# Boese0601/Dyadic-Interaction-Modeling

Measured on AMD Instinct MI355X. Metric: listener clips/sec (T=300, EMOCA-56), higher is better.
Workload: dtype bf16; 1 GPU; C3: B=256/GPU synthetic dyad clips, T=300, SLMFT.forward(mode='val'): listener VQ encode + encoder + 299-step AR decode (top-k 52 sampling) + VQ decode; global_batch=256, seq_len=300, gather=tokens+coeffs, gather_bytes_per_rank=17452032

## Files before the change

dyadic-interaction-modeling_amd/csrc/common.hpp:

```cpp
#pragma once
#include <hip/hip_runtime.h>
#include <stdint.h>
#include <stdio.h>
#include <string.h>
#include <string>

#include "../../include/dimx.h"

namespace dimx {

void set_error(const char* fmt, ...);
const char* get_error();

#define DIMX_HIP(expr)                                                                       \
    do {                                                                                     \
        hipError_t _e = (expr);                                                              \
        if (_e != hipSuccess) {                                                              \
            dimx::set_error("%s:%d: %s -> %s", __FILE__, __LINE__, #expr, hipGetErrorString(_e)); \
            return DIMX_ERR_HIP;                                                             \
        }                                                                                    \
    } while (0)

#define DIMX_REQUIRE(cond, code, ...)       \
    do {                                    \
// ... 362 lines not shown
int lstm_bwd_run(const float* dy, const float* save, const float* const* w_hh, int B, int T, float* dgates, void* scratch,
                 size_t scratch_bytes, int flags, int cu_count, int* fault_count, hipStream_t st);
int launch_context_concat(int out_dtype, const float* x_s, const float* patch, const float* audio, void* ctx,
                          int M, int dim, int dim_a, hipStream_t s);
int launch_finalize_idx(int32_t* idx, const int32_t* lens, int B, int T, int32_t pad_value, hipStream_t s,
                        int fqn = 1);
int launch_shift_tokens(const int32_t* z, int32_t* inp, int32_t* tgt, int B, int T, hipStream_t s);
int launch_ce_argmax(const float* logits, const int32_t* target, float* row_loss, int32_t* argmax_tok, int R,
                     int V, hipStream_t s);
int launch_sample(const float* logits, int ld_logits, int R, int top_k, float temperature, const float* noise,
                  uint64_t seed, const int32_t* step_dev, uint64_t step_host, int32_t* tokens, int tok_ld,
                  int tok_col_from_step, int nslab, long slab_stride, float* logits_out, int logits_out_ld, int row0,
                  int rows_total, const float* emb_table, int emb_C, float* x_next, int32_t* step_rw, unsigned* done_ctr,
                  hipStream_t s, const float* pos_table = nullptr, float pos_scale = 0.f, int pos_rows = 0,
                  const int32_t* dev_params = nullptr,
                  void* y_next = nullptr, const float* y_gamma = nullptr, int y_dtype = DIMX_F32);
int launch_gen_params(int32_t* base, int groups, float temperature, uint64_t seed, int row_off, int rows_total,
                      hipStream_t s);
int launch_embed_step(const float* table, int C, int rows, const int32_t* start, const int32_t* tokens, int tok_ld,
                      const int32_t* step_dev, float* x, int B, int start_div, hipStream_t s,
                      const float* pos_table = nullptr, float pos_scale = 0.f);
int launch_add_pos_rows(float* x, const float* pos, int M, int n, int C, float scale, hipStream_t s);
int launch_mask_lens(const uint8_t* mask, int32_t* lens, int B, int T, hipStream_t s);
int launch_legacy_scramble(int out_dtype, const float* E, const int32_t* idx, const int32_t* lens, void* out, int B,
                           int T, int fqn, int zdim, int n_embed, hipStream_t s);
int launch_step_inc(int32_t* step_dev, hipStream_t s);
int launch_copy_rows_step(const float* src, float* dst, int B, int V, int n, const int32_t* step_dev, hipStream_t s);
int launch_mask_and(const uint8_t* a, const uint8_t* b, uint8_t* out, int n, hipStream_t s);

}
```

dyadic-interaction-modeling_amd/csrc/elementwise.hip:

```cpp
#include "common.hpp"

namespace dimx {
namespace {

template <typename OutT>
__global__ void cast_pad_kernel(const float* __restrict__ x, int ldx, const float* __restrict__ coladd,
                                OutT* __restrict__ y, int ldy, int M, int K, const uint8_t* __restrict__ zero_rows) {
    const long total = (long)M * ldy;
    for (long i = (long)blockIdx.x * blockDim.x + threadIdx.x; i < total; i += (long)gridDim.x * blockDim.x) {
        const int m = (int)(i / ldy), k = (int)(i - (long)m * ldy);
        float v = 0.f;
        if (k < K && !(zero_rows && zero_rows[m])) {
            v = x[(size_t)m * ldx + k];
            if (coladd) v += coladd[k];
        }
        store_from_f32<OutT>(y + i, v);
    }
}

template <typename OutT>
__global__ void gather_rows_kernel(const float* __restrict__ table, int ld_table, int rows,
                                   const int32_t* __restrict__ idx, OutT* __restrict__ y, int ldy, int M, int C) {
    const long total = (long)M * C;
    for (long i = (long)blockIdx.x * blockDim.x + threadIdx.x; i < total; i += (long)gridDim.x * blockDim.x) {
// ... 79 lines not shown
}

__global__ __launch_bounds__(256) void sample_kernel(const float* __restrict__ logits, int ld, int R, int top_k,
                                                     float temperature, const float* __restrict__ noise,
                                                     uint64_t seed, const int32_t* __restrict__ step_dev,
                                                     uint64_t step_host, int32_t* __restrict__ tokens, int tok_ld,
                                                     int tok_col_from_step, int nslab, long slab_stride,
                                                     float* __restrict__ logits_out, int logits_out_ld, int row0,
                                                     int rows_total,
                                                     const float* __restrict__ emb_table, int emb_C,
                                                     float* __restrict__ x_next, int32_t* __restrict__ step_rw,
                                                     unsigned* __restrict__ done_ctr,
                                                     const float* __restrict__ pos_table, float pos_scale,
                                                     int pos_rows, const int32_t* __restrict__ dev_params,
                                                     void* __restrict__ y_next, const float* __restrict__ y_gamma,
                                                     int y_bf16) {
    const int row = blockIdx.x * (blockDim.x >> 6) + (threadIdx.x >> 6), lane = threadIdx.x & 63;
    const uint64_t step = step_dev ? (uint64_t)*step_dev : step_host;
    if (dev_params) {
        temperature = __builtin_bit_cast(float, dev_params[0]);
        seed = *(const uint64_t*)(dev_params + 2);
    }
    const int rng_off = dev_params ? dev_params[4] : 0;
    const int rng_tot = dev_params && dev_params[5] > 0 ? dev_params[5] : rows_total;
    if (row < R) {
    const float* lr = logits + (size_t)row * ld;
    float2 gam[16];
    const bool fast_embed = x_next && emb_C / 2 <= 16 * 64;
    if (y_next && fast_embed) {
#pragma unroll
        for (int k = 0; k < 16; ++k) {
// ... 113 lines not shown
        tok = bi;
    }
    if (lane == 0) tokens[(size_t)row * tok_ld + (tok_col_from_step ? (int)step : 0)] = tok;
    if (x_next) {
        const float2* src = (const float2*)(emb_table + (size_t)tok * emb_C);
        float2* dst = (float2*)(x_next + (size_t)row * emb_C);
        const bool with_pos = pos_table && (int)step + 1 < pos_rows;
        const float2* pr = with_pos ? (const float2*)(pos_table + (size_t)(step + 1) * emb_C) : nullptr;
        const int nv = emb_C / 2;
        if (nv <= 16 * 64) {
            float2 v[16];
#pragma unroll
            for (int k = 0; k < 16; ++k) {
                const int i = lane + 64 * k;
                v[k] = src[i < nv ? i : nv - 1];
            }
            if (with_pos) {
                float2 q[16];
#pragma unroll
                for (int k = 0; k < 16; ++k) {
                    const int i = lane + 64 * k;
                    q[k] = pr[i < nv ? i : nv - 1];
                }
#pragma unroll
                for (int k = 0; k < 16; ++k)
                    v[k] = make_float2(__fadd_rn(v[k].x, __fmul_rn(q[k].x, pos_scale)), __fadd_rn(v[k].y, __fmul_rn(q[k].y, pos_scale)));
            }
#pragma unroll
            for (int k = 0; k < 16; ++k) {
                const int i = lane + 64 * k;
// ... 63 lines not shown
    tok = tok < 0 ? 0 : (tok >= rows ? rows - 1 : tok);
    const float4* src = (const float4*)(table + (size_t)tok * C);
    float4* dst = (float4*)(x + (size_t)b * C);
    if (pos_table) {
        const float4* pr = (const float4*)(pos_table + (size_t)step * C);
        for (int i = threadIdx.x; i < C / 4; i += blockDim.x) {
            const float4 e = src[i], q = pr[i];
            dst[i] = make_float4(__fadd_rn(e.x, __fmul_rn(q.x, pos_scale)), __fadd_rn(e.y, __fmul_rn(q.y, pos_scale)),
                                 __fadd_rn(e.z, __fmul_rn(q.z, pos_scale)), __fadd_rn(e.w, __fmul_rn(q.w, pos_scale)));
        }
    } else {
        for (int i = threadIdx.x; i < C / 4; i += blockDim.x) dst[i] = src[i];
    }
}

__global__ void add_pos_rows_kernel(float* __restrict__ x, const float* __restrict__ pos, int M, int n, int C,
                                    float scale) {
    const long total = (long)M * C;
    for (long i = (long)blockIdx.x * blockDim.x + threadIdx.x; i < total; i += (long)gridDim.x * blockDim.x) {
        const int m = (int)(i / C), c = (int)(i - (long)m * C);
        x[i] = __fadd_rn(x[i], __fmul_rn(pos[(size_t)(m % n) * C + c], scale));
    }
}

__global__ __launch_bounds__(64) void mask_lens_kernel(const uint8_t* __restrict__ mask, int32_t* __restrict__ lens,
                                                       int T) {
    const int b = blockIdx.x;
    int n = 0;
    for (int t = threadIdx.x; t < T; t += 64) n += mask[(size_t)b * T + t] ? 1 : 0;
#pragma unroll
// ... 114 lines not shown

int launch_ce_argmax(const float* logits, const int32_t* target, float* row_loss, int32_t* argmax_tok, int R, int V,
                     hipStream_t s) {
    DIMX_REQUIRE(V == 512, DIMX_ERR_ARG, "ce_argmax: vocabulary %d != 512", V);
    hipLaunchKernelGGL(ce_argmax_kernel, dim3(ceil_div(R, 4)), dim3(256), 0, s, logits, target, row_loss, argmax_tok,
                       R);
    DIMX_HIP(hipGetLastError());
    return DIMX_OK;
}

int launch_sample(const float* logits, int ld_logits, int R, int top_k, float temperature, const float* noise,
                  uint64_t seed, const int32_t* step_dev, uint64_t step_host, int32_t* tokens, int tok_ld,
                  int tok_col_from_step, int nslab, long slab_stride, float* logits_out, int logits_out_ld, int row0,
                  int rows_total, const float* emb_table, int emb_C, float* x_next, int32_t* step_rw, unsigned* done_ctr,
                  hipStream_t s, const float* pos_table, float pos_scale, int pos_rows, const int32_t* dev_params,
                  void* y_next, const float* y_gamma, int y_dtype) {
    DIMX_REQUIRE(logits && tokens && R > 0, DIMX_ERR_ARG, "sample: bad arguments");
    DIMX_REQUIRE(!y_next || (x_next && y_gamma && emb_C % 128 == 0 && emb_C <= 2048), DIMX_ERR_ARG,
                 "sample: the fused pre-norm needs the fused embedding and a width of k * 128 <= 2048");
    const int wpb = R <= 1024 ? 1 : 4;
    hipLaunchKernelGGL(sample_kernel, dim3(ceil_div(R, wpb)), dim3(64 * wpb), 0, s, logits, ld_logits, R, top_k,
                       temperature, noise, seed, step_dev, step_host, tokens, tok_ld, tok_col_from_step, nslab < 1 ? 1 : nslab,
                       slab_stride, logits_out, logits_out_ld, row0, rows_total, emb_table, emb_C, x_next, step_rw, done_ctr,
                       pos_table, pos_scale, pos_rows, dev_params, y_next, y_gamma, y_dtype == DIMX_BF16 ? 1 : 0);
    DIMX_HIP(hipGetLastError());
    return DIMX_OK;
}

int launch_gen_params(int32_t* base, int groups, float temperature, uint64_t seed, int row_off, int rows_total,
                      hipStream_t s) {
    hipLaunchKernelGGL(gen_params_kernel, dim3(1), dim3(64), 0, s, base, groups, temperature, seed, row_off, rows_total);
    DIMX_HIP(hipGetLastError());
    return DIMX_OK;
}

int launch_embed_step(const float* table, int C, int rows, const int32_t* start, const int32_t* tokens, int tok_ld,
                      const int32_t* step_dev, float* x, int B, int start_div, hipStream_t s, const float* pos_table,
                      float pos_scale) {
    DIMX_REQUIRE(C % 4 == 0, DIMX_ERR_ARG, "embed_step: C %% 4");
    hipLaunchKernelGGL(embed_step_kernel, dim3(B), dim3(256), 0, s, table, C, start, tokens, tok_ld, step_dev, x,
                       rows, start_div < 1 ? 1 : start_div, pos_table, pos_scale);
    DIMX_HIP(hipGetLastError());
    return DIMX_OK;
}

int launch_add_pos_rows(float* x, const float* pos, int M, int n, int C, float scale, hipStream_t s) {
    DIMX_REQUIRE(x && pos && M > 0 && n > 0, DIMX_ERR_ARG, "add_pos_rows: bad arguments");
    const long total = (long)M * C;
    const int blocks = (int)(total / 256 + 1 < 4096 ? total / 256 + 1 : 4096);
    hipLaunchKernelGGL(add_pos_rows_kernel, dim3(blocks), dim3(256), 0, s, x, pos, M, n, C, scale);
    DIMX_HIP(hipGetLastError());
    return DIMX_OK;
}

int launch_mask_lens(const uint8_t* mask, int32_t* lens, int B, int T, hipStream_t s) {
    DIMX_REQUIRE(mask && lens && B > 0 && T > 0, DIMX_ERR_ARG, "mask_lens: bad arguments");
// ... 40 lines not shown
```

dyadic-interaction-modeling_amd/csrc/model.hip:

```cpp
#include <stdarg.h>
#include <stdlib.h>
#include <set>

#include "model.hpp"

namespace dimx {

static thread_local char g_err[1024] = "";
void set_error(const char* fmt, ...) {
    va_list ap;
    va_start(ap, fmt);
    vsnprintf(g_err, sizeof(g_err), fmt, ap);
    va_end(ap);
}
const char* get_error() { return g_err; }

static std::string vq_prefix(int which) { return which == 0 ? "speaker_vq." : "listener_vq."; }

struct KeySpec {
    std::string name;
    std::vector<int64_t> shape;
};

static void vq_keys(const dimx_dims& d, int which, std::vector<KeySpec>& out) {
// ... 387 lines not shown
    DIMX_TRY(pack_linear(c, {pre + "project_in.weight"}, c->host.count(pre + "project_in.bias") ? pre + "project_in.bias" : "", false,
                         &e->proj_in));
    DIMX_TRY(upload_f32(c, pre + "pos_emb.emb.weight", &e->pos_emb));
    for (int i = 0; i < c->encg[0].depth; ++i) {
        DIMX_TRY(pack_xattn(c, xl(pre, 2 * i), false, &e->attn[i]));
        DIMX_TRY(pack_xff(c, xl(pre, 2 * i + 1), &e->ff[i]));
    }
    DIMX_TRY(upload_f32(c, pre + "attn_layers.final_norm.weight", &e->final_g));
    return DIMX_OK;
}

static void free_packed(dimx_ctx* c) {
    for (void* p : c->dev_allocs) (void)hipFree(p);
    c->dev_allocs.clear();
    c->packed_mask = 0;
}

enum { COMP_VQ0 = 1, COMP_VQ1 = 2, COMP_ENC = 4, COMP_DEC = 8, COMP_ALL = 15, COMP_MESH = 16 };

static std::vector<KeySpec> comp_keys(const dimx_dims& d, int comp) {
    std::vector<KeySpec> k;
    if (comp == COMP_MESH) {
        mesh_keys(d, k);
        return k;
    }
    if (d.variant == 1) {
        if (comp == COMP_VQ0) legacy_speaker_vq_keys(d, k);
        if (comp == COMP_VQ1) vq_keys(d, 1, k);
        if (comp == COMP_ENC) xenc_keys(d, "generator.encoder.", (int64_t)d.spk_face_quan_num * d.vq_zdim, k);
        if (comp == COMP_DEC) {
// ... 100 lines not shown
        }
        if (comp == COMP_MESH) {
            const std::string p = "vertice_map_reverse_lstm.";
            for (int l = 0; l < 2; ++l)
                for (int dir = 0; dir < 2; ++dir) {
                    const std::string sfx = "_l" + std::to_string(l) + lstm_suffix(dir);
                    DIMX_TRY(upload_f32(c, p + "weight_ih" + sfx, &c->mesh.w_ih[l][dir]));
                    DIMX_TRY(upload_f32(c, p + "weight_hh" + sfx, &c->mesh.w_hh[l][dir]));
                    DIMX_TRY(upload_f32(c, p + "bias_ih" + sfx, &c->mesh.b_ih[l][dir]));
                    DIMX_TRY(upload_f32(c, p + "bias_hh" + sfx, &c->mesh.b_hh[l][dir]));
                }
            DIMX_TRY(pack_linear(c, {"vertice_map_reverse.0.weight"}, "vertice_map_reverse.0.bias", false, &c->mesh.l1));
            DIMX_TRY(pack_linear(c, {"vertice_map_reverse.2.weight"}, "vertice_map_reverse.2.bias", false, &c->mesh.l2));
        }
        c->packed_mask |= comp;
    }
    c->graph_valid = false;
    return DIMX_OK;
}

int vq_pe_buffers(dimx_ctx* c, int which, const float** pe_enc, const float** pe_dec) {
    DIMX_REQUIRE(which == 0 || which == 1, DIMX_ERR_ARG, "vq_pe_buffers: which must be 0 or 1");
    DIMX_HIP(hipSetDevice(c->device));
    DIMX_TRY(ensure_packed(c, which == 0 ? COMP_VQ0 : COMP_VQ1));
    *pe_enc = c->vq[which].pe_enc;
    *pe_dec = c->vq[which].pe_dec;
    return DIMX_OK;
}

static inline size_t es_of(const dimx_ctx* c) { return dtype_size(c->at); }
// ... 263 lines not shown
        c->encg[0] = c->encg[1] = {din, din, d.dim, d.heads, d.dim_head, d.enc_depth, d.ff_mult, 0};
        c->decg = {d.dim, d.heads, d.dim_head, d.dec_depth, d.ff_mult, 1, d.num_tokens, d.dim};
    } else {
        const int causal = d.variant == 2 ? 0 : 1, abs_pos = d.variant == 2 ? 1 : 0;
        c->encg[0] = {d.dim_in, 64, d.dim, d.heads, d.dim_head, d.enc_depth, d.ff_mult, causal};
        c->encg[1] = {d.dim, d.dim, d.dim, d.heads, d.dim_head, d.enc_depth, d.ff_mult, causal};
        c->decg = {d.dim + d.dim_a, d.heads, d.dim_head, d.dec_depth, d.ff_mult, abs_pos, d.num_tokens, d.dim + d.dim_a};
    }
    for (const auto& k : all_keys(d)) c->required.push_back(k.name);
    const char* ng = getenv("DIMX_NO_GRAPH");
    c->use_graph = (ng && ng[0] == '1') ? 0 : 1;
    const char* nc = getenv("DIMX_NO_CHAIN");
    c->use_chain = (nc && nc[0] == '1') ? 0 : 1;
    c->use_layer_chain = getenv("DIMX_NO_LAYER_CHAIN") ? 0 : 1;
    c->multi_tr = getenv("DIMX_NO_MULTI_TR") ? 0 : 1;
    if (getenv("DIMX_LAYER_PROF")) {
        void* p = nullptr;
        if (hipMalloc(&p, (size_t)8 * 256 * 16 * 8) == hipSuccess) {
            (void)hipMemset(p, 0, (size_t)8 * 256 * 16 * 8);
            c->layer_prof_dev = (unsigned long long*)p;
        }
    }
    if (const char* pg = getenv("DIMX_PREFILL_GROUPS")) {
        const int v = atoi(pg);
        if (v >= 1 && v <= dimx_ctx::kPreGroups) c->prefill_groups = v;
    }
    {
        int cus = 0;
        if (hipDeviceGetAttribute(&cus, hipDeviceAttributeMultiprocessorCount, device_id) == hipSuccess) c->cu_count = cus;
    }
// ... 11 lines not shown
        if (h->graph_exec[g]) (void)hipGraphExecDestroy(h->graph_exec[g]);
        if (h->grp_stream[g]) (void)hipStreamDestroy(h->grp_stream[g]);
        if (h->ev_join[g]) (void)hipEventDestroy(h->ev_join[g]);
    }
    if (h->ev_fork) (void)hipEventDestroy(h->ev_fork);
    for (int g = 0; g < dimx_ctx::kPreGroups - 1; ++g) {
        if (h->pre_stream[g]) (void)hipStreamDestroy(h->pre_stream[g]);
        if (h->pre_join[g]) (void)hipEventDestroy(h->pre_join[g]);
    }
    if (h->pre_fork) (void)hipEventDestroy(h->pre_fork);
    if (h->cap_stream) (void)hipStreamDestroy(h->cap_stream);
    if (h->chain_err_ev) (void)hipEventDestroy(h->chain_err_ev);
    if (h->chain_err_dev) (void)hipFree(h->chain_err_dev);
    if (h->chain_stats_dev) (void)hipFree(h->chain_stats_dev);
    if (h->layer_prof_dev) (void)hipFree(h->layer_prof_dev);
    if (h->chain_err_host) (void)hipHostFree(h->chain_err_host);
    free_packed(h);
    train_forget(h);
    delete h;
    return DIMX_OK;
}

int dimx_numeric_mode(dimx_handle h) { return h ? h->mode : DIMX_ERR_ARG; }

int dimx_set_shard(dimx_handle h, int row_offset, int rows_total) {
    DIMX_REQUIRE(h, DIMX_ERR_ARG, "set_shard: null handle");
    DIMX_REQUIRE(row_offset >= 0 && (rows_total == 0 || rows_total > row_offset), DIMX_ERR_ARG,
                 "set_shard: row_offset %d, rows_total %d", row_offset, rows_total);
    h->shard_row_off = row_offset;
    h->shard_rows_total = rows_total;
// ... 871 lines not shown
    const XAttn& sa = h->dec.self_[0];
    const XAttn& ca = h->dec.cross[0];
    c.g1.W = sa.out.w; c.g1.N = sa.out.N; c.g1.K = sa.out.K; c.g1.ldw = sa.out.Kp;
    c.lda1 = dg.heads * dg.dim_head;
    c.g2.W = ca.qkv.w; c.g2.N = ca.qkv.N; c.g2.K = ca.qkv.K; c.g2.ldw = ca.qkv.Kp;
    if (!chain_supported(c, h->cu_count)) return false;
    c.g2.W = h->dec.logits.w; c.g2.N = h->dec.logits.N; c.g2.K = h->dec.logits.K; c.g2.ldw = h->dec.logits.Kp;
    c.g1.W = nullptr;
    return chain_supported(c, h->cu_count) && 3 * dg.depth + 1 <= kChainSites;
}

static bool gen_multi_tr(dimx_handle h, int S) {
    return S > 1 && h->multi_tr && h->at == DIMX_BF16 && h->decg.dim_head == 64;
}

static int gen_step(dimx_handle h, const CtxPersist& cp, const GenScratch& s0, const int32_t* start,
                    const uint8_t* ctx_mask, int row0, int B, int Btot, int grp, int T, float temperature, int top_k,
                    const float* noise, uint64_t seed, int32_t* tokens, float* logits_out, hipStream_t st,
                    bool embed_only = false, int S = 1) {
    const DecGeom& dg = h->decg;
    const int DD = dg.dim, heads = dg.heads, D = dg.dim_head, inner = heads * D;
    const int V = dg.num_tokens, n = gen_steps(h, T), Tp = tpad(T);
    const float* pos = dg.abs_pos ? h->dec.pos_emb : nullptr;
    const float pos_scale = 1.0f / sqrtf((float)DD);
    const size_t es = es_of(h);
    const float scale = 1.0f / sqrtf((float)D);
    GenScratch s = s0;
    auto boff = [&](void* p, size_t per_row_bytes) { return (void*)((unsigned char*)p + (size_t)row0 * per_row_bytes); };
    s.x = s0.x + (size_t)row0 * DD;
    s.y = boff(s0.y, DD * es);
    s.qkv = s0.qkv + (size_t)row0 * 3 * inner;
    s.qc = s0.qc + (size_t)row0 * inner;
    s.xr = s0.xr + (size_t)row0 * DD;
    s.o = boff(s0.o, inner * es);
    s.f = boff(s0.f, (size_t)DD * dg.ff_mult * es);
    s.logits = s0.logits + (size_t)row0 * V;
    s.step = s0.step + 16 * grp;
    const int clip0 = row0 / S, nclip = B / S;
    start += clip0;
    ctx_mask += (size_t)clip0 * T;
    tokens += (size_t)row0 * n;
    if (logits_out) logits_out += (size_t)row0 * n * V;
    if (embed_only) {
        DIMX_TRY(launch_embed_step(h->dec.tok_emb, DD, V, start, tokens, n, s.step, s.x, B, S, st, pos, pos_scale));
        DIMX_TRY(launch_add_slabs_layernorm(h->at, s.x, s.xr, 0, s0.st_xr, s.y, h->dec.self_[0].ln_g, B, DD, st));
        return DIMX_OK;
    }
    auto slab_gemm = [&](const void* A, int lda, const Linear& L, float* out, long stride, int* nsl) -> int {
        GemmArgs g;
        gemm_lin(h, A, lda, L, B, g);
        g.x3_decode = 1;
        g.out_dtype = DIMX_F32;
        g.out_slabs = 1;
        static const bool f32_split = getenv("DIMX_F32_NO_SPLIT") == nullptr;
        if (f32_split) g.allow_splitk = 1;
        g.slab_stride = stride;
        gemm_set_plain_out(g, out, L.N);
        *nsl = gemm_plan_splits(g);
        g.force_splitk = *nsl;
        return launch_gemm(g, st);
    };
    const bool chain = gen_use_chain(h, B, S, grp);
    const bool defer = chain && h->defer_ln && h->chain_stats_dev && h->dec.cross[0].q_ln.w && h->dec.ff[0].f1_ln.w;
    auto chain_site = [&](int site, const void* A1, int lda1, const Linear* W1, int nslab, const float* gamma,
                          const Linear* W2, float* out2, int ld_out2, const float* colsum2 = nullptr) -> int {
        ChainArgs c;
        memset(&c, 0, sizeof(c));
        c.B = B;
        if (defer && W1) {
            c.defer = 1;
            c.stats = h->chain_stats_dev;
            c.colsum2 = colsum2;
        }
        if (W1) {
            c.g1.W = W1->w;
// ... 51 lines not shown
        lc.seen = lc.counters + 8 * 16;
        lc.step = s.step;
        lc.err = h->chain_err_dev;
        lc.fault = h->chain_fault_inject > 0 ? 1 : 0;
        lc.sc_stride = (T + 15) / 16 * 16;
        lc.prof = h->layer_prof_dev ? h->layer_prof_dev + (size_t)l * 256 * 16 : nullptr;
        return true;
    };
    int pending = 0;
    for (int l = 0; l < dg.depth; ++l) {
        GemmArgs g;
        DecodeAttnArgs a;
        int ns = 0;
        if (l > 0)
            DIMX_TRY(launch_add_slabs_layernorm(h->at, s.x, s.xr, pending, s0.st_xr, s.y, h->dec.self_[l].ln_g, B, DD, st));
        DIMX_TRY(slab_gemm(s.y, DD, h->dec.self_[l].qkv, s.qkv, s0.st_qkv, &ns));
        DecodeAttnArgs sa, ca;
        memset(&sa, 0, sizeof(sa));
        sa.dtype = h->at;
        sa.q = s.qkv;
        sa.q_ld = 3 * inner;
        sa.q_f32 = 1;
        sa.nslab = ns;
        sa.slab_stride = s0.st_qkv;
        sa.knew = s.qkv + inner;
        sa.vnew = s.qkv + 2 * inner;
        sa.kv_ld = 3 * inner;
        sa.kcache = boff(s0.sk[l], (size_t)heads * T * 64 * es);
        sa.vcache = boff(s0.sv[l], (size_t)heads * T * 64 * es);
        sa.Tmax = T;
        sa.out = s.o;
// ... 86 lines not shown
        g.act = ACT_GELU_ERF;
        gemm_set_plain_out(g, s.f, DD * dg.ff_mult);
        DIMX_TRY(launch_gemm(g, st));
        DIMX_TRY(slab_gemm(s.f, DD * dg.ff_mult, h->dec.ff[l].f2, s.xr, s0.st_xr, &pending));
    }
    int nlg = 0;
    if (chain && !h->dec.logits.bias) {
        DIMX_TRY(chain_site(3 * dg.depth, nullptr, 0, nullptr, pending, h->dec.final_g, &h->dec.logits, s.logits, V));
        nlg = 1;
    } else {
        DIMX_TRY(launch_add_slabs_layernorm(h->at, s.x, s.xr, pending, s0.st_xr, s.y, h->dec.final_g, B, DD, st));
        DIMX_TRY(slab_gemm(s.y, DD, h->dec.logits, s.logits, s0.st_lg, &nlg));
    }
    DIMX_TRY(launch_sample(s.logits, V, B, top_k, temperature, noise, seed, s.step, 0, tokens, n, 1, nlg, s0.st_lg,
                           logits_out, n, row0, Btot, h->dec.tok_emb, DD, s.x, s.step, (unsigned*)(s.step + 8), st, pos,
                           pos_scale, n, s.step + 2, s.y, h->dec.self_[0].ln_g, h->at));
    return DIMX_OK;
}

}

extern "C" {

static int generate_impl(dimx_handle h, const int32_t* start, const uint8_t* ctx_mask, int B, int T, int n_samples,
                         float temperature, int top_k, const float* exp_noise, uint64_t seed, int32_t* tokens,
                         float* logits_out, void* ws, size_t ws_bytes, void* stream, bool* chain_used) {
    const int S = n_samples < 1 ? 1 : n_samples;
    DIMX_REQUIRE(S == 1 || S == 2 || S == 4 || S == 5 || S == 8 || S == 10, DIMX_ERR_ARG,
                 "generate: n_samples %d not in {1,2,4,5,8,10}", n_samples);
    DIMX_TRY(check_common(h, B, T, ws, ws_bytes, COMP_DEC, S));
    DIMX_REQUIRE(start && ctx_mask && tokens && T >= 2, DIMX_ERR_ARG, "generate: null argument or T < 2");
// ... 11 lines not shown
        DIMX_HIP(hipMalloc((void**)&h->chain_err_dev, 64));
        DIMX_HIP(hipMemset(h->chain_err_dev, 0, 64));
        DIMX_HIP(hipMalloc((void**)&h->chain_stats_dev, 8 * 32 * 32 * 2 * sizeof(float)));
        DIMX_HIP(hipMemset(h->chain_stats_dev, 0, 8 * 32 * 32 * 2 * sizeof(float)));
        DIMX_HIP(hipHostMalloc((void**)&h->chain_err_host, 64, hipHostMallocDefault));
        *h->chain_err_host = 0;
        DIMX_HIP(hipEventCreateWithFlags(&h->chain_err_ev, hipEventDisableTiming));
    }
    DIMX_HIP(hipMemsetAsync(s.chain_ctr, 0, (size_t)kChainSites * kChainSiteWords * 4, st));
    DIMX_TRY(launch_gen_params(s.step, dimx_ctx::kMaxGroups, temperature, seed, h->shard_row_off * S,
                               h->shard_rows_total * S, st));
    if (gen_multi_tr(h, S)) DIMX_TRY(launch_pack_key_words(ctx_mask, T, nullptr, B, T, s.kw, s.kw_cap, st));
    int G = h->gen_groups < 1 ? 1 : h->gen_groups;
    if (G > B) G = B;
    if (S > 1) G = 1;
    int lo[dimx_ctx::kMaxGroups + 1];
    for (int g = 0; g <= G; ++g) lo[g] = (int)((long)R * g / G);
    hipStream_t gs[dimx_ctx::kMaxGroups];
    if (G == 1) {
        gs[0] = st;
    } else {
        if (!h->ev_fork) DIMX_HIP(hipEventCreateWithFlags(&h->ev_fork, hipEventDisableTiming));
        DIMX_HIP(hipEventRecord(h->ev_fork, st));
        for (int g = 0; g < G; ++g) {
            if (!h->grp_stream[g]) DIMX_HIP(hipStreamCreateWithFlags(&h->grp_stream[g], hipStreamNonBlocking));
            if (!h->ev_join[g]) DIMX_HIP(hipEventCreateWithFlags(&h->ev_join[g], hipEventDisableTiming));
            gs[g] = h->grp_stream[g];
            DIMX_HIP(hipStreamWaitEvent(gs[g], h->ev_fork, 0));
        }
    }
    for (int g = 0; g < G; ++g)
        DIMX_TRY(gen_step(h, cp, s, start, ctx_mask, lo[g], lo[g + 1] - lo[g], R, g, T, temperature, top_k, exp_noise,
                          seed, tokens, logits_out, gs[g], true, S));
    if (!h->use_graph) {
        for (int t = 0; t < n; ++t)
            for (int g = 0; g < G; ++g)
                DIMX_TRY(gen_step(h, cp, s, start, ctx_mask, lo[g], lo[g + 1] - lo[g], R, g, T, temperature, top_k,
                                  exp_noise, seed, tokens, logits_out, gs[g], false, S));
    } else {
        GraphKey key{ws, B, T, top_k, 0.f, exp_noise, 0, start, ctx_mask, tokens, logits_out, G * 100 + S + (h->use_chain ? 1000 : 0) + (h->chain_fault_inject > 0 ? 2000 : 0)};
        if (!(h->graph_valid && h->graph_key == key)) {
            h->graph_valid = false;
            if (!h->cap_stream) DIMX_HIP(hipStreamCreateWithFlags(&h->cap_stream, hipStreamNonBlocking));
            for (int g = 0; g < dimx_ctx::kMaxGroups; ++g) {
                if (h->graph_exec[g]) {
                    (void)hipGraphExecDestroy(h->graph_exec[g]);
                    h->graph_exec[g] = nullptr;
                }
                if (h->graph_multi[g]) {
                    (void)hipGraphExecDestroy(h->graph_multi[g]);
                    h->graph_multi[g] = nullptr;
                }
            }
            for (int g = 0; g < G; ++g) {
                for (int pass = 0; pass < 2; ++pass) {
                    const int reps = pass == 0 ? 1 : h->graph_unroll;
                    if (pass == 1 && (reps <= 1 || n < reps)) continue;
                    hipGraph_t graph = nullptr;
                    DIMX_HIP(hipStreamBeginCapture(h->cap_stream, hipStreamCaptureModeThreadLocal));
                    int rc = DIMX_OK;
                    for (int r = 0; r < reps && rc == DIMX_OK; ++r)
                        rc = gen_step(h, cp, s, start, ctx_mask, lo[g], lo[g + 1] - lo[g], R, g, T, temperature, top_k,
                                      exp_noise, seed, tokens, logits_out, h->cap_stream, false, S);
                    const hipError_t ce = hipStreamEndCapture(h->cap_stream, &graph);
                    if (rc != DIMX_OK) {
                        if (graph) (void)hipGraphDestroy(graph);
                        return rc;
                    }
                    DIMX_HIP(ce);
                    DIMX_HIP(hipGraphInstantiate(pass == 0 ? &h->graph_exec[g] : &h->graph_multi[g], graph, nullptr, nullptr, 0));
                    (void)hipGraphDestroy(graph);
                }
            }
            h->graph_key = key;
            h->graph_valid = true;
        }
        {
            const int U = h->graph_unroll;
// ... 84 lines not shown
    if (!e2) return DIMX_OK;
    *h->chain_err_host = 0;
    DIMX_HIP(hipMemsetAsync(h->chain_err_dev, 0, 64, (hipStream_t)stream));
    h->graph_valid = false;
    ++h->chain_faults;
    h->use_chain = 0;
    fprintf(stderr, "dimx: the regenerated batch reported chain flags 0x%x again; regenerating on the one-kernel-per-op step, the "
                    "chain path stays off for this handle\n", e2);
    DIMX_TRY(generate_impl(h, start, ctx_mask, B, T, n_samples, temperature, top_k, exp_noise, seed, tokens, logits_out, ws,
                           ws_bytes, stream, &chain_used));
    DIMX_REQUIRE(!chain_used, DIMX_ERR_STATE, "generate: the chain path is still active after it was switched off");
    return DIMX_OK;
}

int dimx_chain_faults(dimx_handle h) { return h ? h->chain_faults : 0; }

int dimx_lstm_faults(dimx_handle h) { return h ? h->lstm_faults : 0; }

int dimx_mesh_head(dimx_handle h, const float* motion, const float* templ, int B, int L, float* mesh_out, int flags, void* ws,
                   size_t ws_bytes, void* stream) {
    DIMX_REQUIRE(h && h->d.mesh_dim > 0, DIMX_ERR_STATE, "mesh_head: the handle was created without a mesh head (dimx_dims.mesh_dim = 0)");
    DIMX_TRY(check_common(h, B, L, ws, ws_bytes, COMP_MESH));
    DIMX_REQUIRE(motion && mesh_out, DIMX_ERR_ARG, "mesh_head: null argument");
    hipStream_t st = (hipStream_t)stream;
    Arena ar = scratch_arena(h, ws, ws_bytes, B, L, nullptr);
    MeshScratch s;
    plan_mesh(h, ar, B, L, s);
    DIMX_REQUIRE(!ar.overflow, DIMX_ERR_WORKSPACE, "mesh_head: workspace overflow");
    const MeshHead& m = h->mesh;
    const int M = B * L, V = h->d.mesh_dim;
// ... 526 lines not shown
```

dyadic-interaction-modeling_amd/csrc/model.hpp:

```cpp
#pragma once
#include <map>
#include <string>
#include <vector>

#include "common.hpp"

namespace dimx {

struct Linear {
    void* w = nullptr;
    const float* bias = nullptr;
    int N = 0, K = 0, Kp = 0;
    void* w3 = nullptr;
};

struct VQBlock {
    const float *ln1_g, *ln1_b, *ln2_g, *ln2_b;
    Linear qkv, out, l1, l2;
    const void* mlp = nullptr;
};

struct VQNet {
    Linear vm, conv, le, post;
    VQBlock enc[8];
// ... 133 lines not shown
    dimx::GraphKey graph_key{};
    bool graph_valid = false;
    int use_graph = 1;
    int use_chain = 1;
    int cu_count = 0;
    float* chain_stats_dev = nullptr;
    int defer_ln = 1;
    unsigned long long* layer_prof_dev = nullptr;
    int multi_tr = 1;
    int use_layer_chain = 1;
    unsigned* chain_err_dev = nullptr;
    unsigned* chain_err_host = nullptr;
    hipEvent_t chain_err_ev = nullptr;
    int chain_faults = 0;
    int chain_fault_inject = 0;
    int shard_row_off = 0, shard_rows_total = 0;
    dimx::MeshHead mesh;
    int lstm_faults = 0;
    int spk_embed_rows = 0;
};
```

dyadic-interaction-modeling_amd/engine.py:

```python
import ctypes

import numpy as np
import torch

from . import lib as L


class Engine:
    def __init__(self, device=None, mode=L.MODE_PARITY_F32, variant="slmft", mesh_dim=0):
        if not torch.cuda.is_available():
            raise L.DimxError("dimx needs a ROCm GPU (torch.cuda.is_available() is False); "
                              "there is no CPU fallback")
        self.device = torch.device(device if device is not None else "cuda:0")
        if self.device.index is None:
            self.device = torch.device("cuda", torch.cuda.current_device())
        self.lib = L.load()
        self.mode = mode
        assert variant in ("slmft", "legacy", "slm", "speaker")
        self.variant = variant
        if variant == "speaker":
            assert mesh_dim > 0, "the speaker variant needs mesh_dim"
            self.dims = L.speaker_dims(mesh_dim)
        else:
            self.dims = {"slmft": L.default_dims, "legacy": L.legacy_dims, "slm": L.slm_dims}[variant]()
# ... 208 lines not shown
            assert tuple(template.shape) == (B, V), "template must be [B, mesh_dim]"
        if out is None:
            out = torch.empty(B, Lq, V, dtype=torch.float32, device=self.device)
        assert tuple(out.shape) == (B, Lq, V) and out.dtype == torch.float32
        self._chk(motion, template, out)
        ws, wsb = self.workspace(B, Lq)
        L.check(self.lib.dimx_mesh_head(self.h, L.ptr(motion), L.ptr(template), B, Lq, L.ptr(out), 1 if safe else 0, ws, wsb,
                                        self._s()), "dimx_mesh_head")
        return out

    def lstm_faults(self):
        return int(self.lib.dimx_lstm_faults(self.h))

    def chain_faults(self):
        return int(self.lib.dimx_chain_faults(self.h))

    def debug_chain_fault(self, n_calls=1):
        L.check(self.lib.dimx_debug_chain_fault(self.h, int(n_calls)), "dimx_debug_chain_fault")


def _pad_k(w, mult):
    N, K = w.shape
    Kp = (K + mult - 1) // mult * mult
    if Kp == K:
        return w.contiguous()
    out = torch.zeros(N, Kp, dtype=w.dtype, device=w.device)
    out[:, :K] = w
    return out


# ... 511 lines not shown
```

dyadic-interaction-modeling_amd/lib.py:

```python
import ctypes
import os
from ctypes import (POINTER, c_char_p, c_float, c_int, c_int32, c_int64, c_size_t, c_uint64,
                    c_void_p)

import torch

HERE = os.path.dirname(os.path.abspath(__file__))
LIB_PATH = os.environ.get("DIMX_LIB", os.path.join(HERE, "libdimx_hip.so"))

MODE_PARITY_F32 = 0
MODE_PERF_BF16 = 1
F32, BF16 = 0, 1
ACT_NONE, ACT_LEAKY, ACT_GELU_TANH, ACT_GELU_ERF = 0, 1, 2, 3


class DimxError(RuntimeError):
    pass


class Dims(ctypes.Structure):
    _fields_ = [(n, c_int) for n in (
        "vq_in_dim", "vq_hidden", "vq_layers", "vq_heads", "vq_inter", "vq_n_embed", "vq_zdim",
        "dim_in", "dim", "dim_a", "enc_depth", "dec_depth", "heads", "dim_head", "num_tokens",
        "max_seq_len", "ff_mult", "variant", "spk_in_dim", "spk_hidden", "spk_heads", "spk_inter",
# ... 66 lines not shown
    "dimx_train_spk_num_params": (c_int, [c_void_p]),
    "dimx_train_spk_total": (c_int64, [c_void_p]),
    "dimx_train_spk_param_info": (c_int, [c_void_p, c_int, POINTER(c_char_p), POINTER(c_int64), POINTER(c_int64)]),
    "dimx_train_spk_workspace_bytes": (c_size_t, [c_void_p, c_int, c_int]),
    "dimx_train_spk_forward_backward": (c_int, [c_void_p] + [c_void_p] * 9 + [c_int, c_int, c_void_p, c_void_p, c_void_p, c_void_p, c_void_p,
                                                c_size_t, c_void_p]),
    "dimx_op_lstm_layer_bwd": (c_int, [c_int, c_void_p, c_int, c_int, c_int, c_int, POINTER(c_void_p), POINTER(c_void_p),
                                       POINTER(c_void_p), POINTER(c_void_p), c_void_p, c_void_p, POINTER(c_void_p), POINTER(c_void_p),
                                       POINTER(c_void_p), c_int, POINTER(c_int), c_void_p]),
    "dimx_train_adamw": (c_int, [c_void_p, c_void_p, c_void_p, c_void_p, c_int64, c_float, c_float, c_float, c_float, c_float,
                                 c_int, c_float, c_void_p, c_void_p]),
    "dimx_op_train_attention": (c_int, [c_int, c_void_p, c_void_p, c_void_p, c_void_p, c_void_p, c_void_p, c_int, c_int, c_int,
                                        c_int, c_int, c_float, c_void_p, c_void_p, c_void_p, c_void_p, c_void_p, c_void_p,
                                        c_void_p]),
    "dimx_chain_faults": (c_int, [c_void_p]),
    "dimx_lstm_faults": (c_int, [c_void_p]),
    "dimx_mesh_head": (c_int, [c_void_p, c_void_p, c_void_p, c_int, c_int, c_void_p, c_int, c_void_p, c_size_t, c_void_p]),
    "dimx_op_lstm_layer": (c_int, [c_int, c_void_p, c_int, c_int, c_int, c_int, POINTER(c_void_p), POINTER(c_void_p),
                                   POINTER(c_void_p), POINTER(c_void_p), c_void_p, c_int, POINTER(c_int), c_void_p]),
    "dimx_debug_chain_fault": (c_int, [c_void_p, c_int]),
    "dimx_op_gemm_slabs": (c_int, [c_int, c_int, c_int, c_int, c_int]),
    "dimx_op_split_x3": (c_int, [c_void_p, c_void_p, ctypes.c_long, c_void_p]),
    "dimx_op_gemm_x3": (c_int, [c_void_p, c_int, c_void_p, c_void_p, c_int, c_int, c_int, c_int, c_void_p, c_int, c_void_p, c_int, c_int,
                                c_void_p]),
    "dimx_op_gemm": (c_int, [c_int, c_int, c_void_p, c_int, c_void_p, c_int, c_void_p, c_int, c_int, c_int,
                             c_int, c_void_p, c_int, c_void_p, c_int, c_int, c_void_p, c_int, c_void_p]),
    "dimx_op_gemm_headmajor": (c_int, [c_int, c_void_p, c_int, c_void_p, c_int, c_void_p, c_int, c_int, c_int, c_int, c_int,
                                       c_int, c_void_p]),
    "dimx_op_layernorm": (c_int, [c_int, c_void_p, c_void_p, c_void_p, c_void_p, c_int, c_int, c_void_p]),
    "dimx_op_instnorm": (c_int, [c_int, c_void_p, c_void_p, c_void_p, c_int, c_int, c_int, c_void_p]),
# ... 129 lines not shown
```

include/dimx.h:

```cpp
#ifndef DIMX_H
#define DIMX_H

#include <stddef.h>
#include <stdint.h>

#ifdef __cplusplus
extern "C" {
#endif

typedef struct dimx_ctx* dimx_handle;

typedef enum {
    DIMX_OK = 0,
    DIMX_ERR_ARG = -1,
    DIMX_ERR_HIP = -2,
    DIMX_ERR_WEIGHT = -3,
    DIMX_ERR_STATE = -4,
    DIMX_ERR_WORKSPACE = -5
} dimx_status;

#define DIMX_MODE_PARITY_F32 0
#define DIMX_MODE_PERF_BF16 1

#define DIMX_F32 0
// ... 60 lines not shown
                     int T, int for_generate, void* ws, size_t ws_bytes, void* stream);

int dimx_legacy_speaker_features(dimx_handle h, const float* v_speaker, const uint8_t* mask, int B, int T,
                                 float* x_speaker_out, int32_t* idx_out, void* ws, size_t ws_bytes,
                                 void* stream);

int dimx_decode_tf(dimx_handle h, const int32_t* z_l, const uint8_t* ctx_mask, const uint8_t* kv_mask,
                   int B, int T, float* logits, float* row_loss, int32_t* argmax_tok, void* ws,
                   size_t ws_bytes, void* stream);

int dimx_generate(dimx_handle h, const int32_t* start, const uint8_t* ctx_mask, int B, int T, int n_samples,
                  float temperature, int top_k, const float* exp_noise, uint64_t seed, int32_t* tokens,
                  float* logits_out, void* ws, size_t ws_bytes, void* stream);

int dimx_chain_faults(dimx_handle h);
int dimx_debug_chain_fault(dimx_handle h, int n_calls);

int dimx_mesh_head(dimx_handle h, const float* motion, const float* templ, int B, int L, float* mesh_out, int flags, void* ws,
                   size_t ws_bytes, void* stream);
int dimx_lstm_faults(dimx_handle h);

int dimx_train_num_params(dimx_handle h);
int64_t dimx_train_total(dimx_handle h);
int dimx_train_param_info(dimx_handle h, int i, const char** name, int64_t* offset, int64_t* numel);
size_t dimx_train_workspace_bytes(dimx_handle h, int B, int T);
int dimx_train_forward_backward(dimx_handle h, const float* params, float* grads, const float* v_speaker, const float* v_audio,
                                const uint8_t* mask, const int32_t* z_l, const uint8_t* kv_mask, int B, int T, float* loss_out,
                                float* logits_out, void* ws, size_t ws_bytes, void* stream);
int dimx_train_graph_stats(dimx_handle h, int64_t* out3);
size_t dimx_train_legacy_workspace_bytes(dimx_handle h, int B, int T);
// ... 118 lines not shown
```

Baseline: 1675 clips/s.

## Precompute layer-0 QKV per vocabulary token and gather it during AR decode

Layer 0's self-attention input depends only on the sampled token (no absolute positional term), so the token embedding, first layernorm and QKV projection are precomputed once for every vocabulary entry into a cached table. The table is invalidated by a decoder-weight epoch. The sampler then copies the table row for each sampled token straight into the QKV buffer, and the per-step layer-0 layernorm and QKV GEMM are skipped. This trades a one-time build and V*3*inner floats of memory for removing one GEMM and one norm from each of the 299 decode steps. The path only applies with a single group and no absolute positions.

```diff
diff --git a/dyadic-interaction-modeling_amd/csrc/common.hpp b/dyadic-interaction-modeling_amd/csrc/common.hpp
--- a/dyadic-interaction-modeling_amd/csrc/common.hpp
+++ b/dyadic-interaction-modeling_amd/csrc/common.hpp
@@ -400,7 +400,13 @@
                   int rows_total, const float* emb_table, int emb_C, float* x_next, int32_t* step_rw, unsigned* done_ctr,
                   hipStream_t s, const float* pos_table = nullptr, float pos_scale = 0.f, int pos_rows = 0,
                   const int32_t* dev_params = nullptr,
-                  void* y_next = nullptr, const float* y_gamma = nullptr, int y_dtype = DIMX_F32);
+                  void* y_next = nullptr, const float* y_gamma = nullptr, int y_dtype = DIMX_F32,
+                  const float* qkv0_table = nullptr, float* qkv0_out = nullptr, int qkv0_N = 0);
+int launch_iota_clamp(int32_t* ids, int n, int rows, hipStream_t s);
+int launch_sum_slabs_rows(const float* slabs, int nslab, long slab_stride, float* table, int id0, int rows, int M, int N,
+                          hipStream_t s);
+int launch_gather_start_rows(const float* table, int N, int rows, const int32_t* start, int start_div, float* out, int B,
+                             hipStream_t s);
 int launch_gen_params(int32_t* base, int groups, float temperature, uint64_t seed, int row_off, int rows_total,
                       hipStream_t s);
 int launch_embed_step(const float* table, int C, int rows, const int32_t* start, const int32_t* tokens, int tok_ld,
diff --git a/dyadic-interaction-modeling_amd/csrc/elementwise.hip b/dyadic-interaction-modeling_amd/csrc/elementwise.hip
--- a/dyadic-interaction-modeling_amd/csrc/elementwise.hip
+++ b/dyadic-interaction-modeling_amd/csrc/elementwise.hip
@@ -117,7 +117,8 @@
                                                      const float* __restrict__ pos_table, float pos_scale,
                                                      int pos_rows, const int32_t* __restrict__ dev_params,
                                                      void* __restrict__ y_next, const float* __restrict__ y_gamma,
-                                                     int y_bf16) {
+                                                     int y_bf16, const float* __restrict__ qkv0_table,
+                                                     float* __restrict__ qkv0_out, int qkv0_N) {
     const int row = blockIdx.x * (blockDim.x >> 6) + (threadIdx.x >> 6), lane = threadIdx.x & 63;
     const uint64_t step = step_dev ? (uint64_t)*step_dev : step_host;
     if (dev_params) {
@@ -261,6 +262,23 @@
             for (int k = 0; k < 16; ++k) {
                 const int i = lane + 64 * k;
                 v[k] = src[i < nv ? i : nv - 1];
+            }
+            if (qkv0_table) {
+                const float4* qs = (const float4*)(qkv0_table + (size_t)tok * qkv0_N);
+                float4* qd = (float4*)(qkv0_out + (size_t)row * qkv0_N);
+                const int nq = qkv0_N / 4;
+                float4 w[12];
+#pragma unroll
+                for (int k = 0; k < 12; ++k) {
+                    const int i = lane + 64 * k;
+                    w[k] = make_float4(0.f, 0.f, 0.f, 0.f);
+                    if (i < nq) w[k] = qs[i];
+                }
+#pragma unroll
+                for (int k = 0; k < 12; ++k) {
+                    const int i = lane + 64 * k;
+                    if (i < nq) qd[i] = w[k];
+                }
             }
             if (with_pos) {
                 float2 q[16];
@@ -354,6 +372,38 @@
     }
 }
 
+__global__ void iota_clamp_kernel(int32_t* __restrict__ ids, int n, int rows) {
+    const int i = blockIdx.x * blockDim.x + threadIdx.x;
+    if (i < n) ids[i] = i < rows ? i : rows - 1;
+}
+
+__global__ __launch_bounds__(256) void sum_slabs_rows_kernel(const float* __restrict__ slabs, int nslab, long slab_stride,
+                                                             float* __restrict__ table, int id0, int rows, int M, int N) {
+    const int m = blockIdx.x;
+    if (m >= M || id0 + m >= rows) return;
+    const float4* src = (const float4*)(slabs + (size_t)m * N);
+    float4* dst = (float4*)(table + (size_t)(id0 + m) * N);
+    for (int i = threadIdx.x; i < N / 4; i += blockDim.x) {
+        float4 v = src[i];
+        for (int s = 1; s < nslab; ++s) {
+            const float4 t = *(const float4*)(slabs + (size_t)s * slab_stride + (size_t)m * N + 4 * i);
+            v.x = __fadd_rn(v.x, t.x); v.y = __fadd_rn(v.y, t.y); v.z = __fadd_rn(v.z, t.z); v.w = __fadd_rn(v.w, t.w);
+        }
+        dst[i] = v;
+    }
+}
+
+__global__ __launch_bounds__(256) void gather_start_rows_kernel(const float* __restrict__ table, int N, int rows,
+                                                                const int32_t* __restrict__ start, int start_div,
+                                                                float* __restrict__ out) {
+    const int b = blockIdx.x;
+    int tok = start[b / start_div];
+    tok = tok < 0 ? 0 : (tok >= rows ? rows - 1 : tok);
+    const float4* src = (const float4*)(table + (size_t)tok * N);
+    float4* dst = (float4*)(out + (size_t)b * N);
+    for (int i = threadIdx.x; i < N / 4; i += blockDim.x) dst[i] = src[i];
+}
+
 __global__ void add_pos_rows_kernel(float* __restrict__ x, const float* __restrict__ pos, int M, int n, int C,
                                     float scale) {
     const long total = (long)M * C;
@@ -498,15 +548,19 @@
                   int tok_col_from_step, int nslab, long slab_stride, float* logits_out, int logits_out_ld, int row0,
                   int rows_total, const float* emb_table, int emb_C, float* x_next, int32_t* step_rw, unsigned* done_ctr,
                   hipStream_t s, const float* pos_table, float pos_scale, int pos_rows, const int32_t* dev_params,
-                  void* y_next, const float* y_gamma, int y_dtype) {
+                  void* y_next, const float* y_gamma, int y_dtype, const float* qkv0_table, float* qkv0_out, int qkv0_N) {
     DIMX_REQUIRE(logits && tokens && R > 0, DIMX_ERR_ARG, "sample: bad arguments");
+    DIMX_REQUIRE(!qkv0_table || (x_next && qkv0_out && !pos_table && emb_C / 2 <= 16 * 64 && qkv0_N % 4 == 0 && qkv0_N > 0 &&
+                                 qkv0_N <= 12 * 256),
+                 DIMX_ERR_ARG, "sample: the q/k/v table rides on the fused embedding (no positional table) and holds rows of k * 4 <= 3072");
     DIMX_REQUIRE(!y_next || (x_next && y_gamma && emb_C % 128 == 0 && emb_C <= 2048), DIMX_ERR_ARG,
                  "sample: the fused pre-norm needs the fused embedding and a width of k * 128 <= 2048");
     const int wpb = R <= 1024 ? 1 : 4;
     hipLaunchKernelGGL(sample_kernel, dim3(ceil_div(R, wpb)), dim3(64 * wpb), 0, s, logits, ld_logits, R, top_k,
                        temperature, noise, seed, step_dev, step_host, tokens, tok_ld, tok_col_from_step, nslab < 1 ? 1 : nslab,
                        slab_stride, logits_out, logits_out_ld, row0, rows_total, emb_table, emb_C, x_next, step_rw, done_ctr,
-                       pos_table, pos_scale, pos_rows, dev_params, y_next, y_gamma, y_dtype == DIMX_BF16 ? 1 : 0);
+                       pos_table, pos_scale, pos_rows, dev_params, y_next, y_gamma, y_dtype == DIMX_BF16 ? 1 : 0, qkv0_table,
+                       qkv0_out, qkv0_N);
     DIMX_HIP(hipGetLastError());
     return DIMX_OK;
 }
@@ -524,6 +578,30 @@
     DIMX_REQUIRE(C % 4 == 0, DIMX_ERR_ARG, "embed_step: C %% 4");
     hipLaunchKernelGGL(embed_step_kernel, dim3(B), dim3(256), 0, s, table, C, start, tokens, tok_ld, step_dev, x,
                        rows, start_div < 1 ? 1 : start_div, pos_table, pos_scale);
+    DIMX_HIP(hipGetLastError());
+    return DIMX_OK;
+}
+
+int launch_iota_clamp(int32_t* ids, int n, int rows, hipStream_t s) {
+    DIMX_REQUIRE(ids && n > 0 && rows > 0, DIMX_ERR_ARG, "iota_clamp: bad arguments");
+    hipLaunchKernelGGL(iota_clamp_kernel, dim3(ceil_div(n, 256)), dim3(256), 0, s, ids, n, rows);
+    DIMX_HIP(hipGetLastError());
+    return DIMX_OK;
+}
+
+int launch_sum_slabs_rows(const float* slabs, int nslab, long slab_stride, float* table, int id0, int rows, int M, int N,
+                          hipStream_t s) {
+    DIMX_REQUIRE(slabs && table && nslab >= 1 && M > 0 && N > 0 && N % 4 == 0 && slab_stride % 4 == 0 && id0 >= 0, DIMX_ERR_ARG,
+                 "sum_slabs_rows: bad arguments");
+    hipLaunchKernelGGL(sum_slabs_rows_kernel, dim3(M), dim3(256), 0, s, slabs, nslab, slab_stride, table, id0, rows, M, N);
+    DIMX_HIP(hipGetLastError());
+    return DIMX_OK;
+}
+
+int launch_gather_start_rows(const float* table, int N, int rows, const int32_t* start, int start_div, float* out, int B,
+                             hipStream_t s) {
+    DIMX_REQUIRE(table && start && out && B > 0 && N > 0 && N % 4 == 0 && rows > 0, DIMX_ERR_ARG, "gather_start_rows: bad arguments");
+    hipLaunchKernelGGL(gather_start_rows_kernel, dim3(B), dim3(256), 0, s, table, N, rows, start, start_div < 1 ? 1 : start_div, out);
     DIMX_HIP(hipGetLastError());
     return DIMX_OK;
 }
diff --git a/dyadic-interaction-modeling_amd/csrc/model.hip b/dyadic-interaction-modeling_amd/csrc/model.hip
--- a/dyadic-interaction-modeling_amd/csrc/model.hip
+++ b/dyadic-interaction-modeling_amd/csrc/model.hip
@@ -425,6 +425,7 @@
     for (void* p : c->dev_allocs) (void)hipFree(p);
     c->dev_allocs.clear();
     c->packed_mask = 0;
+    ++c->dec_epoch;
 }
 
 enum { COMP_VQ0 = 1, COMP_VQ1 = 2, COMP_ENC = 4, COMP_DEC = 8, COMP_ALL = 15, COMP_MESH = 16 };
@@ -555,6 +556,7 @@
             DIMX_TRY(pack_linear(c, {"vertice_map_reverse.2.weight"}, "vertice_map_reverse.2.bias", false, &c->mesh.l2));
         }
         c->packed_mask |= comp;
+        if (comp == COMP_DEC) ++c->dec_epoch;
     }
     c->graph_valid = false;
     return DIMX_OK;
@@ -848,6 +850,7 @@
     c->use_chain = (nc && nc[0] == '1') ? 0 : 1;
     c->use_layer_chain = getenv("DIMX_NO_LAYER_CHAIN") ? 0 : 1;
     c->multi_tr = getenv("DIMX_NO_MULTI_TR") ? 0 : 1;
+    c->use_qkv0_table = getenv("DIMX_NO_QKV0_TABLE") ? 0 : 1;
     if (getenv("DIMX_LAYER_PROF")) {
         void* p = nullptr;
         if (hipMalloc(&p, (size_t)8 * 256 * 16 * 8) == hipSuccess) {
@@ -889,6 +892,7 @@
     if (h->chain_err_dev) (void)hipFree(h->chain_err_dev);
     if (h->chain_stats_dev) (void)hipFree(h->chain_stats_dev);
     if (h->layer_prof_dev) (void)hipFree(h->layer_prof_dev);
+    if (h->qkv0_table) (void)hipFree(h->qkv0_table);
     if (h->chain_err_host) (void)hipHostFree(h->chain_err_host);
     free_packed(h);
     train_forget(h);
@@ -1790,10 +1794,59 @@
     return S > 1 && h->multi_tr && h->at == DIMX_BF16 && h->decg.dim_head == 64;
 }
 
+static int slab_gemm_rows(dimx_handle h, int B, hipStream_t st, const void* A, int lda, const Linear& L, float* out, long stride,
+                          int* nsl) {
+    GemmArgs g;
+    gemm_lin(h, A, lda, L, B, g);
+    g.x3_decode = 1;
+    g.out_dtype = DIMX_F32;
+    g.out_slabs = 1;
+    static const bool f32_split = getenv("DIMX_F32_NO_SPLIT") == nullptr;
+    if (f32_split) g.allow_splitk = 1;
+    g.slab_stride = stride;
+    gemm_set_plain_out(g, out, L.N);
+    *nsl = gemm_plan_splits(g);
+    g.force_splitk = *nsl;
+    return launch_gemm(g, st);
+}
+
+static bool qkv0_table_supported(dimx_handle h) {
+    const DecGeom& dg = h->decg;
+    const int N = 3 * dg.heads * dg.dim_head;
+    return h->use_qkv0_table && !dg.abs_pos && h->dec.self_[0].qkv.N == N && N % 4 == 0 && N <= 12 * 256 && dg.dim % 4 == 0 &&
+           dg.dim / 2 <= 16 * 64;
+}
+
+static int qkv0_table_build(dimx_handle h, const GenScratch& s, int M, hipStream_t st) {
+    const DecGeom& dg = h->decg;
+    const int DD = dg.dim, V = dg.num_tokens, N = h->dec.self_[0].qkv.N;
+    if (h->qkv0_table && h->qkv0_M == M && h->qkv0_at == h->at && h->qkv0_epoch == h->dec_epoch) return DIMX_OK;
+    if (!h->qkv0_table) {
+        DIMX_HIP(hipMalloc((void**)&h->qkv0_table, (size_t)V * N * sizeof(float)));
+        h->graph_valid = false;
+    }
+    h->qkv0_epoch = 0;
+    const int rounds = (V + M - 1) / M;
+    int32_t* ids = (int32_t*)s.logits;
+    DIMX_TRY(launch_iota_clamp(ids, rounds * M, V, st));
+    for (int r = 0; r < rounds; ++r) {
+        int ns = 0;
+        DIMX_TRY(launch_embed_step(h->dec.tok_emb, DD, V, ids + (size_t)r * M, nullptr, 0, s.step, s.x, M, 1, st));
+        DIMX_TRY(launch_add_slabs_layernorm(h->at, s.x, s.xr, 0, s.st_xr, s.y, h->dec.self_[0].ln_g, M, DD, st));
+        DIMX_TRY(slab_gemm_rows(h, M, st, s.y, DD, h->dec.self_[0].qkv, s.qkv, s.st_qkv, &ns));
+        DIMX_TRY(launch_sum_slabs_rows(s.qkv, ns, s.st_qkv, h->qkv0_table, r * M, V, M, N, st));
+    }
+    h->qkv0_M = M;
+    h->qkv0_at = h->at;
+    h->qkv0_epoch = h->dec_epoch;
+    ++h->qkv0_builds;
+    return DIMX_OK;
+}
+
 static int gen_step(dimx_handle h, const CtxPersist& cp, const GenScratch& s0, const int32_t* start,
                     const uint8_t* ctx_mask, int row0, int B, int Btot, int grp, int T, float temperature, int top_k,
                     const float* noise, uint64_t seed, int32_t* tokens, float* logits_out, hipStream_t st,
-                    bool embed_only = false, int S = 1) {
+                    bool embed_only = false, int S = 1, const float* qkv0 = nullptr) {
     const DecGeom& dg = h->decg;
     const int DD = dg.dim, heads = dg.heads, D = dg.dim_head, inner = heads * D;
     const int V = dg.num_tokens, n = gen_steps(h, T), Tp = tpad(T);
@@ -1819,22 +1872,14 @@
     if (logits_out) logits_out += (size_t)row0 * n * V;
     if (embed_only) {
         DIMX_TRY(launch_embed_step(h->dec.tok_emb, DD, V, start, tokens, n, s.step, s.x, B, S, st, pos, pos_scale));
-        DIMX_TRY(launch_add_slabs_layernorm(h->at, s.x, s.xr, 0, s0.st_xr, s.y, h->dec.self_[0].ln_g, B, DD, st));
+        if (qkv0)
+            DIMX_TRY(launch_gather_start_rows(qkv0, 3 * inner, V, start, S, s.qkv, B, st));
+        else
+            DIMX_TRY(launch_add_slabs_layernorm(h->at, s.x, s.xr, 0, s0.st_xr, s.y, h->dec.self_[0].ln_g, B, DD, st));
         return DIMX_OK;
     }
     auto slab_gemm = [&](const void* A, int lda, const Linear& L, float* out, long stride, int* nsl) -> int {
-        GemmArgs g;
-        gemm_lin(h, A, lda, L, B, g);
-        g.x3_decode = 1;
-        g.out_dtype = DIMX_F32;
-        g.out_slabs = 1;
-        static const bool f32_split = getenv("DIMX_F32_NO_SPLIT") == nullptr;
-        if (f32_split) g.allow_splitk = 1;
-        g.slab_stride = stride;
-        gemm_set_plain_out(g, out, L.N);
-        *nsl = gemm_plan_splits(g);
-        g.force_splitk = *nsl;
-        return launch_gemm(g, st);
+        return slab_gemm_rows(h, B, st, A, lda, L, out, stride, nsl);
     };
     const bool chain = gen_use_chain(h, B, S, grp);
     const bool defer = chain && h->defer_ln && h->chain_stats_dev && h->dec.cross[0].q_ln.w && h->dec.ff[0].f1_ln.w;
@@ -1916,7 +1961,10 @@
         int ns = 0;
         if (l > 0)
             DIMX_TRY(launch_add_slabs_layernorm(h->at, s.x, s.xr, pending, s0.st_xr, s.y, h->dec.self_[l].ln_g, B, DD, st));
-        DIMX_TRY(slab_gemm(s.y, DD, h->dec.self_[l].qkv, s.qkv, s0.st_qkv, &ns));
+        if (l == 0 && qkv0)
+            ns = 1;
+        else
+            DIMX_TRY(slab_gemm(s.y, DD, h->dec.self_[l].qkv, s.qkv, s0.st_qkv, &ns));
         DecodeAttnArgs sa, ca;
         memset(&sa, 0, sizeof(sa));
         sa.dtype = h->at;
@@ -2033,7 +2081,8 @@
     }
     DIMX_TRY(launch_sample(s.logits, V, B, top_k, temperature, noise, seed, s.step, 0, tokens, n, 1, nlg, s0.st_lg,
                            logits_out, n, row0, Btot, h->dec.tok_emb, DD, s.x, s.step, (unsigned*)(s.step + 8), st, pos,
-                           pos_scale, n, s.step + 2, s.y, h->dec.self_[0].ln_g, h->at));
+                           pos_scale, n, s.step + 2, qkv0 ? nullptr : s.y, qkv0 ? nullptr : h->dec.self_[0].ln_g, h->at, qkv0,
+                           s.qkv, 3 * inner));
     return DIMX_OK;
 }
 
@@ -2075,6 +2124,11 @@
     int G = h->gen_groups < 1 ? 1 : h->gen_groups;
     if (G > B) G = B;
     if (S > 1) G = 1;
+    const float* qkv0 = nullptr;
+    if (G == 1 && qkv0_table_supported(h)) {
+        DIMX_TRY(qkv0_table_build(h, s, R, st));
+        qkv0 = h->qkv0_table;
+    }
     int lo[dimx_ctx::kMaxGroups + 1];
     for (int g = 0; g <= G; ++g) lo[g] = (int)((long)R * g / G);
     hipStream_t gs[dimx_ctx::kMaxGroups];
@@ -2092,14 +2146,14 @@
     }
     for (int g = 0; g < G; ++g)
         DIMX_TRY(gen_step(h, cp, s, start, ctx_mask, lo[g], lo[g + 1] - lo[g], R, g, T, temperature, top_k, exp_noise,
-                          seed, tokens, logits_out, gs[g], true, S));
+                          seed, tokens, logits_out, gs[g], true, S, qkv0));
     if (!h->use_graph) {
         for (int t = 0; t < n; ++t)
             for (int g = 0; g < G; ++g)
                 DIMX_TRY(gen_step(h, cp, s, start, ctx_mask, lo[g], lo[g + 1] - lo[g], R, g, T, temperature, top_k,
-                                  exp_noise, seed, tokens, logits_out, gs[g], false, S));
+                                  exp_noise, seed, tokens, logits_out, gs[g], false, S, qkv0));
     } else {
-        GraphKey key{ws, B, T, top_k, 0.f, exp_noise, 0, start, ctx_mask, tokens, logits_out, G * 100 + S + (h->use_chain ? 1000 : 0) + (h->chain_fault_inject > 0 ? 2000 : 0)};
+        GraphKey key{ws, B, T, top_k, 0.f, exp_noise, 0, start, ctx_mask, tokens, logits_out, G * 100 + S + (h->use_chain ? 1000 : 0) + (h->chain_fault_inject > 0 ? 2000 : 0) + (qkv0 ? 4000 : 0)};
         if (!(h->graph_valid && h->graph_key == key)) {
             h->graph_valid = false;
             if (!h->cap_stream) DIMX_HIP(hipStreamCreateWithFlags(&h->cap_stream, hipStreamNonBlocking));
@@ -2122,7 +2176,7 @@
                     int rc = DIMX_OK;
                     for (int r = 0; r < reps && rc == DIMX_OK; ++r)
                         rc = gen_step(h, cp, s, start, ctx_mask, lo[g], lo[g + 1] - lo[g], R, g, T, temperature, top_k,
-                                      exp_noise, seed, tokens, logits_out, h->cap_stream, false, S);
+                                      exp_noise, seed, tokens, logits_out, h->cap_stream, false, S, qkv0);
                     const hipError_t ce = hipStreamEndCapture(h->cap_stream, &graph);
                     if (rc != DIMX_OK) {
                         if (graph) (void)hipGraphDestroy(graph);
@@ -2237,6 +2291,7 @@
 }
 
 int dimx_chain_faults(dimx_handle h) { return h ? h->chain_faults : 0; }
+int dimx_qkv0_table_builds(dimx_handle h) { return h ? h->qkv0_builds : 0; }
 
 int dimx_lstm_faults(dimx_handle h) { return h ? h->lstm_faults : 0; }
 
diff --git a/dyadic-interaction-modeling_amd/csrc/model.hpp b/dyadic-interaction-modeling_amd/csrc/model.hpp
--- a/dyadic-interaction-modeling_amd/csrc/model.hpp
+++ b/dyadic-interaction-modeling_amd/csrc/model.hpp
@@ -171,6 +171,12 @@
     hipEvent_t chain_err_ev = nullptr;
     int chain_faults = 0;
     int chain_fault_inject = 0;
+    int use_qkv0_table = 1;
+    float* qkv0_table = nullptr;
+    int qkv0_M = 0, qkv0_at = -1;
+    uint64_t qkv0_epoch = 0;
+    uint64_t dec_epoch = 1;
+    int qkv0_builds = 0;
     int shard_row_off = 0, shard_rows_total = 0;
     dimx::MeshHead mesh;
     int lstm_faults = 0;
diff --git a/dyadic-interaction-modeling_amd/engine.py b/dyadic-interaction-modeling_amd/engine.py
--- a/dyadic-interaction-modeling_amd/engine.py
+++ b/dyadic-interaction-modeling_amd/engine.py
@@ -246,6 +246,9 @@
 
     def chain_faults(self):
         return int(self.lib.dimx_chain_faults(self.h))
+
+    def qkv0_table_builds(self):
+        return int(self.lib.dimx_qkv0_table_builds(self.h))
 
     def debug_chain_fault(self, n_calls=1):
         L.check(self.lib.dimx_debug_chain_fault(self.h, int(n_calls)), "dimx_debug_chain_fault")
diff --git a/dyadic-interaction-modeling_amd/lib.py b/dyadic-interaction-modeling_amd/lib.py
--- a/dyadic-interaction-modeling_amd/lib.py
+++ b/dyadic-interaction-modeling_amd/lib.py
@@ -104,6 +104,7 @@
                                         c_int, c_int, c_float, c_void_p, c_void_p, c_void_p, c_void_p, c_void_p, c_void_p,
                                         c_void_p]),
     "dimx_chain_faults": (c_int, [c_void_p]),
+    "dimx_qkv0_table_builds": (c_int, [c_void_p]),
     "dimx_lstm_faults": (c_int, [c_void_p]),
     "dimx_mesh_head": (c_int, [c_void_p, c_void_p, c_void_p, c_int, c_int, c_void_p, c_int, c_void_p, c_size_t, c_void_p]),
     "dimx_op_lstm_layer": (c_int, [c_int, c_void_p, c_int, c_int, c_int, c_int, POINTER(c_void_p), POINTER(c_void_p),
diff --git a/include/dimx.h b/include/dimx.h
--- a/include/dimx.h
+++ b/include/dimx.h
@@ -98,6 +98,7 @@
                   float* logits_out, void* ws, size_t ws_bytes, void* stream);
 
 int dimx_chain_faults(dimx_handle h);
+int dimx_qkv0_table_builds(dimx_handle h);
 int dimx_debug_chain_fault(dimx_handle h, int n_calls);
 
 int dimx_mesh_head(dimx_handle h, const float* motion, const float* templ, int B, int L, float* mesh_out, int flags, void* ws,
```

Result: faster. 1696 clips/s (median of 6 runs) (+1.3%).
